# zifuwan/Sigma

Hardware: AMD Instinct MI355X
Metric: images/sec fwd+bwd sigma_small 480x640 (higher is better)
Workload: dtype f32

## Files before the change

### include/sigma_ops.h

```cpp
#ifndef SIGMA_OPS_H_
#define SIGMA_OPS_H_

#include <stdint.h>

#ifdef __cplusplus
extern "C" {
#endif

enum sigma_ops_status {
    SIGMA_OPS_OK = 0,
    SIGMA_OPS_ERR_ARG = 1,
    SIGMA_OPS_ERR_LAUNCH = 5
};

typedef struct sigma_dwconv_params {
    int32_t batch, channels, height, width;
    int32_t n_orders;
    int32_t flags;
    const float *x;
    const float *weight;
    const float *bias;
    float *out2;
    const float *g2;
    float *gpre;
// ... 79 lines not shown
    float *dbeta;
    float *workspace;
    const float *gate;
    int64_t gate_row_stride;
    float *dgate;
    int64_t dgate_row_stride;
    const float *row_scale;
    int64_t rows_per_scale;
    const float *dx_add;
} sigma_layernorm_params;

int sigma_layernorm_fwd(const sigma_layernorm_params *params, void *stream);
int sigma_layernorm_bwd(const sigma_layernorm_params *params, void *stream);
int sigma_layernorm_bwd_partial_rows(int64_t rows, int32_t channels);

typedef struct sigma_seg_accumulate_params {
    int64_t pixels;
    int32_t classes;
    int32_t first;
    const float *score;
    double *acc;
    int64_t score_plane_stride;
    int64_t acc_plane_stride;
} sigma_seg_accumulate_params;

int sigma_seg_accumulate(const sigma_seg_accumulate_params *params, void *stream);

typedef struct sigma_seg_confusion_params {
    int64_t pixels;
    int32_t classes;
// ... 19 lines not shown
```

### sigma_amd/_capi.py

```python
from __future__ import annotations

import ctypes
import os
from typing import Optional

_HERE = os.path.dirname(os.path.abspath(__file__))
LIB_PATH = os.environ.get("SIGMA_HIP_LIB") or os.path.join(_HERE, "lib", "libsigma_hip.so")

SIGMA_SCAN_ABI_VERSION = 12
SIGMA_SCAN_CHUNK = 2048
SIGMA_SCAN_CKPT_PITCH = 1280
SIGMA_SCAN_CKPT_PITCH_FINE = 640
SIGMA_SCAN_CKPT_PITCH_320 = 320
SIGMA_SCAN_CKPT_PITCH_160 = 160
SIGMA_SCAN_CKPT_PITCH_16 = 16
SIGMA_SCAN_MAX_DSTATE = 256
SIGMA_SCAN_BWD_DETERMINISTIC = 1
SIGMA_DWCONV_DETERMINISTIC = 1

DTYPE_F32, DTYPE_F16, DTYPE_BF16 = 0, 1, 2


class SigmaHipUnavailable(RuntimeError):
    pass
# ... 68 lines not shown

class LayerNormParams(ctypes.Structure):
    _fields_ = [
        ("rows", ctypes.c_int64), ("channels", ctypes.c_int32), ("eps", ctypes.c_float),
        ("x", ctypes.c_void_p), ("gamma", ctypes.c_void_p), ("beta", ctypes.c_void_p),
        ("y", ctypes.c_void_p), ("mean", ctypes.c_void_p), ("rstd", ctypes.c_void_p),
        ("dy", ctypes.c_void_p), ("dx", ctypes.c_void_p), ("dgamma", ctypes.c_void_p), ("dbeta", ctypes.c_void_p),
        ("workspace", ctypes.c_void_p),
        ("gate", ctypes.c_void_p), ("gate_row_stride", ctypes.c_int64), ("dgate", ctypes.c_void_p),
        ("dgate_row_stride", ctypes.c_int64),
        ("row_scale", ctypes.c_void_p), ("rows_per_scale", ctypes.c_int64),
        ("dx_add", ctypes.c_void_p),
    ]


class GemmParams(ctypes.Structure):
    _fields_ = [
        ("M", ctypes.c_int64), ("N", ctypes.c_int32), ("K", ctypes.c_int32),
        ("A", ctypes.c_void_p), ("Bt", ctypes.c_void_p), ("C", ctypes.c_void_p), ("bias", ctypes.c_void_p),
        ("lda", ctypes.c_int64), ("ldb", ctypes.c_int64), ("ldc", ctypes.c_int64),
        ("accumulate", ctypes.c_int32), ("batch", ctypes.c_int32),
        ("strideA", ctypes.c_int64), ("strideB", ctypes.c_int64), ("strideC", ctypes.c_int64),
        ("a_mod", ctypes.c_int32), ("pieces", ctypes.c_int32),
        ("c_mod", ctypes.c_int32), ("reserved", ctypes.c_int32),
        ("residual", ctypes.c_void_p), ("residual2", ctypes.c_void_p), ("ldr", ctypes.c_int64), ("strideR", ctypes.c_int64),
        ("Ct", ctypes.c_void_p), ("ldct", ctypes.c_int64), ("t_cols", ctypes.c_int32), ("k_slices", ctypes.c_int32),
        ("workspace", ctypes.c_void_p), ("workspace_bytes", ctypes.c_int64),
    ]


# ... 12 lines not shown
        ("score_plane_stride", ctypes.c_int64), ("acc_plane_stride", ctypes.c_int64),
    ]


class SegConfusionParams(ctypes.Structure):
    _fields_ = [
        ("pixels", ctypes.c_int64), ("classes", ctypes.c_int32), ("n_cl", ctypes.c_int32),
        ("gt_elem_size", ctypes.c_int32), ("pred_elem_size", ctypes.c_int32),
        ("acc", ctypes.c_void_p), ("acc_plane_stride", ctypes.c_int64),
        ("pred", ctypes.c_void_p), ("gt", ctypes.c_void_p), ("hist", ctypes.c_void_p), ("counts", ctypes.c_void_p),
    ]


SIGMA_CE_BLOCKS = 1024
SIGMA_SEG_LDS_HIST_BYTES = 32768

GEMM_SYMBOLS = ("sigma_gemm_nt_split3", "sigma_gemm_nn_split3", "sigma_gemm_tn_split3")
GEMM_AUX_SYMBOLS = ("sigma_gemm_selftest", "sigma_gemm_workspace_bytes", "sigma_gemm_plan")
GEMM_FORMS = {"nt": 0, "nn": 1, "tn": 2}
GEMM_EPILOGUES = ("rows", "direct", "transposed")
GEMM_RES_LOADS = ("none", "vector", "scalar")
GEMM_STORES = ("store", "accumulate", "atomic")

OPS_SYMBOLS = ("sigma_dwconv3x3_silu_fwd", "sigma_dwconv3x3_silu_bwd", "sigma_cross_merge_nhwc", "sigma_cross_split_nhwc",
               "sigma_layernorm_fwd", "sigma_layernorm_bwd", "sigma_layernorm_bwd_partial_rows", "sigma_transpose2d",
               "sigma_pair_sum_add", "sigma_upsample2x_nhwc", "sigma_plane_pool", "sigma_plane_scale",
               "sigma_plane_dot", "sigma_plane_gate_bwd", "sigma_softmax_ce_fwd", "sigma_softmax_ce_bwd", "sigma_colscale_bwd",
               "sigma_colscale_bwd_ws", "sigma_seg_accumulate", "sigma_seg_argmax_confusion")
OPS_AUX_SYMBOLS = ("sigma_dwconv3x3_silu_bwd_workspace_bytes", "sigma_colscale_bwd_workspace_bytes")

EXPORTED_SYMBOLS = (
    "sigma_selective_scan_fwd",
    "sigma_selective_scan_bwd",
    "sigma_scan_bwd_workspace_bytes",
    "sigma_scan_fwd_workspace_bytes",
    "sigma_scan_last_error",
    "sigma_scan_abi_version",
    "sigma_scan_set_option",
    "sigma_scan_get_option",
    "sigma_scan_fwd_plan",
    "sigma_scan_bwd_plan",
    "sigma_scan_selftest",
    "sigma_scan_rowlane_selftest",
)
# ... 57 lines not shown
            fn.argtypes = [ctypes.c_void_p, ctypes.c_void_p, ctypes.c_void_p, ctypes.c_void_p, ctypes.c_void_p, ctypes.c_int64,
                           ctypes.c_int32, ctypes.c_void_p]
        elif name == "sigma_colscale_bwd_ws":
            fn.argtypes = [ctypes.c_void_p, ctypes.c_void_p, ctypes.c_void_p, ctypes.c_void_p, ctypes.c_void_p, ctypes.c_int64,
                           ctypes.c_int32, ctypes.c_void_p, ctypes.c_int64, ctypes.c_void_p]
        elif name == "sigma_softmax_ce_fwd":
            fn.argtypes = [ctypes.c_void_p, ctypes.c_void_p, ctypes.c_int64, ctypes.c_int32, ctypes.c_int64, ctypes.c_void_p,
                           ctypes.c_void_p, ctypes.c_void_p]
        elif name == "sigma_softmax_ce_bwd":
            fn.argtypes = [ctypes.c_void_p, ctypes.c_void_p, ctypes.c_void_p, ctypes.c_void_p, ctypes.c_int64, ctypes.c_int32,
                           ctypes.c_int64, ctypes.c_void_p, ctypes.c_void_p]
        elif name == "sigma_seg_accumulate":
            fn.argtypes = [P(SegAccumulateParams), ctypes.c_void_p]
        elif name == "sigma_seg_argmax_confusion":
            fn.argtypes = [P(SegConfusionParams), ctypes.c_void_p]
        else:
            st = (MergeParams if "cross_" in name else LayerNormParams if "layernorm" in name else
                  TransposeParams if "transpose" in name else DwConvParams)
            fn.argtypes = [P(st), ctypes.c_void_p]
        fn.restype = ctypes.c_int
    lib.sigma_dwconv3x3_silu_bwd_workspace_bytes.argtypes = [P(DwConvParams)]
    lib.sigma_dwconv3x3_silu_bwd_workspace_bytes.restype = ctypes.c_int64
    lib.sigma_colscale_bwd_workspace_bytes.argtypes = [ctypes.c_int64, ctypes.c_int32]
    lib.sigma_colscale_bwd_workspace_bytes.restype = ctypes.c_int64
    for name in GEMM_SYMBOLS:
        fn = getattr(lib, name)
        fn.argtypes = [P(GemmParams), ctypes.c_void_p]
        fn.restype = ctypes.c_int
    lib.sigma_gemm_selftest.argtypes = [ctypes.c_void_p]
    lib.sigma_gemm_selftest.restype = ctypes.c_int
    lib.sigma_gemm_workspace_bytes.argtypes = [P(GemmParams), ctypes.c_int]
    lib.sigma_gemm_workspace_bytes.restype = ctypes.c_int64
    lib.sigma_gemm_plan.argtypes = [P(GemmParams), ctypes.c_int, P(ctypes.c_int32 * 8)]
    lib.sigma_gemm_plan.restype = ctypes.c_int
    if lib.sigma_scan_abi_version() != SIGMA_SCAN_ABI_VERSION:
        raise SigmaHipUnavailable(
            f"ABI mismatch: library {lib.sigma_scan_abi_version()} vs binding {SIGMA_SCAN_ABI_VERSION}; rebuild")
    _lib = lib
    return lib
# ... 29 lines not shown
```

### sigma_amd/build.py

```python
from __future__ import annotations

import argparse
import concurrent.futures as cf
import os
import subprocess
import sys

HERE = os.path.dirname(os.path.abspath(__file__))
CSRC = os.path.join(HERE, "csrc")
OBJ = os.path.join(HERE, "lib", "obj")
LIB = os.path.join(HERE, "lib", "libsigma_hip.so")
SOURCES = ["scan_fwd.hip", "scan_fwd4.hip", "scan_fwdr.hip", "scan_bwdr.hip", "scan_bwd.hip", "scan_bwd2.hip", "scan_bwd3.hip", "scan_bwd4.hip", "selftest.hip", "capi.hip", "dwconv.hip", "merge.hip", "layernorm.hip", "gemm_split.hip", "upsample.hip", "pointwise.hip", "segmetric.hip"]
HEADERS = ["scan_device.h", "scan_launch.h", "scan_quad.h", "scan_rowlane.h", os.path.join("..", "..", "include", "sigma_scan.h"),
           os.path.join("..", "..", "include", "sigma_ops.h"), os.path.join("..", "..", "include", "sigma_gemm.h")]
HIPCC = os.environ.get("HIPCC", "/opt/rocm/bin/hipcc")
FLAGS = [
    "--offload-arch=gfx950", "-O3", "-std=c++17", "-fPIC",
    "-munsafe-fp-atomics",
    "-ffp-contract=off",
    "-fno-slp-vectorize",
    "-Wall", "-Wno-unused-function",
]


def _newer(target: str, deps) -> bool:
    if not os.path.exists(target):
        return True
# ... 45 lines not shown
```

### sigma_amd/selective_scan_cuda_core.py

```python
from __future__ import annotations

import ctypes
from typing import List, Optional

import torch

from . import _capi

_DTYPES = {torch.float32: _capi.DTYPE_F32, torch.float16: _capi.DTYPE_F16, torch.bfloat16: _capi.DTYPE_BF16}


_launch_hook = None


def set_launch_hook(hook) -> None:
    global _launch_hook
    _launch_hook = hook


def _launch(kind, key, fn):
    return fn() if _launch_hook is None else _launch_hook(kind, key, fn)


def _check(cond: bool, msg: str) -> None:
# ... 178 lines not shown
        stream = torch.cuda.current_stream(u.device).cuda_stream
        key = (batch, dim, seqlen, dstate, sizes[4], u.element_size())
        _launch("fwd", key, lambda: _capi.check(
            lib.sigma_selective_scan_fwd(ctypes.byref(fp), ctypes.c_void_p(stream)), "selective_scan_fwd"))
    return [out, x]


def bwd(u: torch.Tensor, delta: torch.Tensor, A: torch.Tensor, B: torch.Tensor, C: torch.Tensor,
        D_: Optional[torch.Tensor], delta_bias_: Optional[torch.Tensor], dout: torch.Tensor,
        x_: Optional[torch.Tensor], delta_softplus: bool, nrows: int) -> List[Optional[torch.Tensor]]:
    return bwd_ext(u, delta, A, B, C, D_, delta_bias_, dout, x_, delta_softplus, nrows=nrows)


def bwd_ext(u, delta, A, B, C, D_, delta_bias_, dout, x_, delta_softplus, nrows: int = 1, rev_mask: int = 0,
            u_gshift: int = 0, dout_gshift: int = 0, dB_out: Optional[torch.Tensor] = None,
            dC_out: Optional[torch.Tensor] = None, ckpt_pitch: int = 0, param_swap: int = 0) -> List[Optional[torch.Tensor]]:
    lib = _capi.load()
    sizes = _check_common(u, delta, A, B, C, D_, delta_bias_, nrows, u_gshift)
    batch, dim, seqlen, dstate, n_groups = sizes
    _check(dout.dtype == u.dtype, "dout must have the dtype of u")
    _check(dout.is_cuda, "dout must be a GPU tensor")
    _check(tuple(dout.shape) == (batch, dim >> dout_gshift, seqlen), "dout must have shape (batch_size, dim, seqlen)")
    _check(dout.stride(-1) == 1 or seqlen <= 1, "dout.stride(-1) must be 1")
    if ckpt_pitch == _capi.SIGMA_SCAN_CKPT_PITCH_16 and batch > 0 and seqlen > 0 and (
            dout.data_ptr() % 16 != 0 or any(s % 4 != 0 for s in dout.stride()[:-1])):
        dout = dout.contiguous()
        if dout.data_ptr() % 16 != 0:
            dout = dout.clone()
    n_chunks = (seqlen + _capi.SIGMA_SCAN_CHUNK - 1) // _capi.SIGMA_SCAN_CHUNK
    if n_chunks > 1 or seqlen > _capi.SIGMA_SCAN_CKPT_PITCH:
        _check(x_ is not None, "x is required when seqlen > 2048")
    if x_ is not None:
        _check(x_.dtype == torch.float32 and x_.is_cuda and x_.is_contiguous(), "x must be a contiguous float32 GPU tensor")
        if x_.dim() == 3:
            pitch = _fine_pitch(x_, seqlen, dstate, ckpt_pitch)
            _check(tuple(x_.shape) == (batch, dim, _ckpt_slots(seqlen, pitch) * dstate), "fine-checkpoint x must be (batch, dim, ceil(L/pitch)*dstate)")
        else:
            _check(tuple(x_.shape) == (batch, dim, n_chunks, 2 * dstate),
                   "x must have shape (batch_size, dim, n_chunks, 2 * dstate)")
    du = torch.empty_like(delta)
    ddelta = torch.empty_like(delta)
    det = torch.are_deterministic_algorithms_enabled()
    if det and batch > 0 and seqlen > 0:
        zeros = torch.empty(dim * dstate + 2 * dim, dtype=torch.float32, device=A.device)
    else:
        zeros = torch.zeros(dim * dstate + 2 * dim, dtype=torch.float32, device=A.device)
    dA = zeros[:dim * dstate].view(dim, dstate)
    if dB_out is not None:
        _check(dB_out.dtype == torch.float32 and tuple(dB_out.shape) == tuple(B.shape) and dB_out.stride(-1) == 1 and
               dC_out is not None and dC_out.dtype == torch.float32 and tuple(dC_out.shape) == tuple(C.shape) and
               dC_out.stride(-1) == 1, "dB_out / dC_out must be fp32 views shaped like B / C")
        dB, dC = dB_out, dC_out
    elif batch > 0 and seqlen > 0:
        dB = torch.empty(B.shape, dtype=torch.float32, device=B.device)
        dC = torch.empty(C.shape, dtype=torch.float32, device=C.device)
    else:
        dB, dC = torch.zeros_like(B, dtype=torch.float32), torch.zeros_like(C, dtype=torch.float32)
    dD = zeros[dim * dstate:dim * dstate + dim] if D_ is not None else None
    ddelta_bias = zeros[dim * dstate + dim:] if delta_bias_ is not None else None
    if batch > 0 and seqlen > 0:
        bp = _capi.BwdParams()
# ... 20 lines not shown
            key = (batch, dim, seqlen, dstate, n_groups, u.element_size())
            _launch("bwd", key, lambda: _capi.check(
                lib.sigma_selective_scan_bwd(ctypes.byref(bp), ctypes.c_void_p(stream)), "selective_scan_bwd"))
            if (ckpt_pitch == _capi.SIGMA_SCAN_CKPT_PITCH_16 and lib.sigma_scan_get_option(b"rl_chain") == 2
                    and not torch.cuda.is_current_stream_capturing()):
                n = lib.sigma_scan_get_option(b"rl_chain_timeouts")
                if n != 0:
                    raise RuntimeError(
                        f"selective_scan_bwd: {n if n > 0 else 'an unknown number of'} hand-over wait(s) of the chained "
                        "row-lane walk ran out (the producer workgroup was not resident: another stream's kernel held "
                        "its slot); the gradients of this call hold NaN. Unset the 'rl_chain' option or run the scan "
                        "alone on the device")
    if dB_out is None:
        dB, dC = dB.to(B.dtype), dC.to(C.dtype)
    return [du, ddelta, dA, dB, dC, dD, ddelta_bias]
```

### sigma_amd/ss2d_fused.py

```python
from __future__ import annotations

import torch

import os as _os_early

from . import gemm as _gemm
from ._handoff import claim_xz_grad_buffer
from . import selective_scan_cuda_core as _core

_PERM = (0, 2, 1, 3)
_REV_MASK = 0b1010
_XPROJ_ALL = _os_early.environ.get("SIGMA_GEMM_XPROJ", "") == "all"
_XPROJ = 0 if _gemm.gemm_mode() == "fp32" else (2 if _XPROJ_ALL else _gemm._pieces("SIGMA_GEMM_XPROJ", "2"))


def _perm4(t: torch.Tensor) -> torch.Tensor:
    return t.unflatten(0, (2, 2)).transpose(0, 1).flatten(0, 1)
import os as _os
_CKPT_ENV = _os.environ.get("SIGMA_CKPT_PITCH", "auto")


def rowlane_possible() -> bool:
    return _CKPT_ENV in ("auto", "16")


def rowlane_pays(seqlen: int, dstate: int, rows: int, groups: int) -> bool:
    if seqlen < 600:
        return False
# ... 177 lines not shown
        if pair_sum:
            Bsz, dim, L = out.shape
            if B.shape[1] != 2:
                raise RuntimeError("pair_sum: two groups only")
            o4 = out.view(Bsz, 2, dim // 2, L)
            return o4[:, 0] + o4[:, 1]
        return out

    @staticmethod
    def backward(ctx, dout):
        u, delta, A, B, C, D, delta_bias, ck = ctx.saved_tensors
        rev_mask, sh, pair_sum = ctx.ext
        dout = dout.float()
        if dout.stride(-1) != 1:
            dout = dout.contiguous()
        du, ddelta, dA, dB, dC, dD, dbias = _core.bwd_ext(u, delta, A, B, C, D, delta_bias, dout, ck,
                                                          True, rev_mask=rev_mask, u_gshift=sh, dout_gshift=1 if pair_sum else 0,
                                                          ckpt_pitch=ctx.pitch)
        if sh:
            Bsz, dim, L = du.shape
            G = B.shape[1]
            rpg = dim // G
            du = du.view(Bsz, G >> sh, 1 << sh, rpg, L).sum(2).reshape(Bsz, dim >> sh, L)
        return du, ddelta, dA.clone(), dB, dC, dD.clone(), dbias.clone(), None, None, None


def selective_scan_ext(u, delta, A, B, C, D, delta_bias, rev_mask=0, u_gshift=0, pair_sum=False):
    return SelectiveScanExtFn.apply(u, delta, A, B, C, D, delta_bias, rev_mask, u_gshift, pair_sum)


def _merge_params(B, d, H, W):
    from . import _capi
    p = _capi.MergeParams()
    p.batch, p.channels, p.height, p.width = B, d, H, W
    return p


def cross_merge_nhwc(ys: torch.Tensor, H: int, W: int) -> torch.Tensor:
    import ctypes
# ... 93 lines not shown
        if L != H * W:
            raise RuntimeError("SS2DCoreFn: xs2 must be (B, 2, d, H*W)")
        K, c, _ = x_proj_weight.shape
        R = dt_projs_weight.shape[2]
        N = A_logs.shape[1]
        if K != 4:
            raise RuntimeError("SS2DCoreFn expects the 4-direction parameter stack")
        xs2 = xs2.float().contiguous()
        Wst, WstT, dtw, A = _derived_params(x_proj_weight, dt_projs_weight, A_logs)
        legal = bool(_XPROJ) and L % 4 == 0 and d % 4 == 0 and c % 2 == 0
        short = L <= 600 or _XPROJ_ALL
        mid = L <= 1200 or _XPROJ_ALL
        own_x = legal
        own_dt = legal and R % 4 == 0 and mid
        ctx.own = dict(xd=legal, xw=legal and mid, dd=legal and R % 4 == 0 and _XPROJ_ALL, dw=legal and R % 4 == 0 and short)
        if own_x:
            p4 = torch.empty((B, 4, c, L), device=xs2.device, dtype=torch.float32)
            _gemm.bgemm_nn(Wst, xs2.view(2 * B, d, L), p4.view(2 * B, 2 * c, L), pieces=_XPROJ)
        else:
            p4 = torch.matmul(Wst.unsqueeze(0), xs2).view(B, 4, c, L)
        if own_dt:
            delta = torch.empty((B, 4, d, L), device=xs2.device, dtype=torch.float32)
            _gemm.bgemm_nn(dtw, p4.view(4 * B, c, L)[:, :R], delta.view(4 * B, d, L), pieces=_XPROJ)
        else:
            delta = torch.matmul(dtw.unsqueeze(0), p4[:, :, :R])
        Dp = Ds.float()
        bias = dt_projs_bias.float().reshape(-1)
        Bv, Cv = p4[:, :, R:R + N], p4[:, :, R + N:]
        need_x = any(ctx.needs_input_grad)
        u2, dl2 = xs2.view(B, 2 * d, L), delta.view(B, 4 * d, L)
# ... 3 lines not shown
        ctx.pitch = pitch
        y = cross_merge_nhwc(out.view(B, 4, d, L), H, W)
        ctx.save_for_backward(xs2, p4, delta, A, Dp, bias, ck, Wst, dtw, WstT)
        ctx.dims = (B, d, H, W, c, R, N)
        return y

    @staticmethod
    def backward(ctx, dy):
        xs2, p4, delta, A, Dp, bias, ck, Wst, dtw, WstT = ctx.saved_tensors
        B, d, H, W, c, R, N = ctx.dims
        own = ctx.own
        L = H * W
        g2 = cross_split_nhwc(dy.float().contiguous())
        dp4 = torch.empty_like(p4)
        Bv, Cv = p4[:, :, R:R + N], p4[:, :, R + N:]
        du, ddelta, dA, _, _, dD, dbias = _core.bwd_ext(
            xs2.view(B, 2 * d, L), delta.view(B, 4 * d, L), A, Bv, Cv, Dp, bias, g2.view(B, 2 * d, L), ck, True,
            rev_mask=_REV_MASK, u_gshift=1, dout_gshift=1, dB_out=dp4[:, :, R:R + N], dC_out=dp4[:, :, R + N:], param_swap=1,
            ckpt_pitch=ctx.pitch)
        ddelta4 = ddelta.view(B, 4, d, L)
        wg = torch.empty(4 * d * R + 4 * c * d, device=xs2.device, dtype=torch.float32) if (own["xw"] or own["dw"]) else None
        if own["dd"]:
            _gemm.bgemm_nn(dtw.transpose(1, 2).contiguous(), ddelta.view(4 * B, d, L), dp4.view(4 * B, c, L)[:, :R], pieces=_XPROJ)
        else:
            dp4[:, :, :R] = torch.matmul(dtw.transpose(1, 2).unsqueeze(0), ddelta4)
        if own["dw"]:
            d_dtw = wg[:4 * d * R].view(4, d, R)
            _gemm.bgemm_nt_sum(ddelta.view(4 * B, d, L), p4.view(4 * B, c, L)[:, :R], d_dtw, pieces=_XPROJ, accumulate=False)
        else:
            d_dtw = torch.matmul(ddelta4, p4[:, :, :R].transpose(-1, -2)).sum(0)
        dp2 = dp4.view(B, 2, 2 * c, L)
        if own["xd"]:
            dxs2 = torch.empty((B, 2, d, L), device=xs2.device, dtype=torch.float32)
            du3 = du.view(2 * B, 2, d, L)
            _gemm.bgemm_nn(WstT, dp4.view(2 * B, 2 * c, L), dxs2.view(2 * B, d, L),
                           residual=du3[:, 0], residual2=du3[:, 1], pieces=_XPROJ)
        else:
            dxs2 = torch.matmul(WstT.unsqueeze(0), dp2)
            _pair_sum_add(du, dxs2, B * 2, d * L)
        if own["xw"]:
            dWst = wg[4 * d * R:].view(2, 2 * c, d)
            _gemm.bgemm_nt_sum(dp4.view(2 * B, 2 * c, L), xs2.view(2 * B, d, L), dWst, pieces=_XPROJ, accumulate=False)
        else:
            dWst = torch.matmul(dp2, xs2.transpose(-1, -2)).sum(0)
        d_xproj = _perm4(dWst.view(4, c, d))
        d_dtw = _perm4(d_dtw)
        dA_logs = dA * A
        dDs = dD.clone()
        dbias = dbias.clone().view(4, d)
        return dxs2, None, None, d_xproj, d_dtw, dbias, dA_logs, dDs


class _TwoOrdersFn(torch.autograd.Function):

    @staticmethod
    def forward(ctx, x):
        ctx.hw = x.shape[2:]
        return _two_orders(x.float())

    @staticmethod
    def backward(ctx, g):
        H, W = ctx.hw
        B, _, d, L = g.shape
        return g[:, 0].reshape(B, d, H, W) + g[:, 1].reshape(B, d, W, H).transpose(2, 3)

# ... 9 lines not shown
```

Measured before the change: 49.88.

## Fuse dt-projection backward GEMMs and scan parameter-grad epilogue into HIP kernels

Adds a dtproj backward kernel that computes both ddt (dtw^T·ddelta) and d_dtw (ddelta·dt^T) from a single pass over ddelta using MFMA, with a split-row reduction stage. It also adds a scan_param_grads kernel that fuses dA*A, the dD/dbias copies, the four-way permutations, and zeroing of a borrowed accumulator buffer into one launch, replacing several small torch ops and clones. The fused dtproj path is enabled only when seqlen >= 4800 by default. This adds workspace and extra code paths, and requires careful cleanup of the borrowed accumulator when an error occurs.

Result: no change. 50.21, median of 6 (+0.7%).

```diff
diff --git a/include/sigma_ops.h b/include/sigma_ops.h
--- a/include/sigma_ops.h
+++ b/include/sigma_ops.h
@@ -117,6 +117,46 @@
 int sigma_layernorm_bwd(const sigma_layernorm_params *params, void *stream);
 int sigma_layernorm_bwd_partial_rows(int64_t rows, int32_t channels);
 
+#define SIGMA_DTPROJ_LBLOCK 256
+#define SIGMA_DTPROJ_MAX_RANK 48
+#define SIGMA_DTPROJ_TARGET_WGS 1280
+typedef struct sigma_dtproj_bwd_params {
+    int32_t batch, groups, dim, seqlen;
+    int32_t rank, reserved_;
+    const float *ddelta;
+    const float *dt;
+    const float *dtw;
+    float *ddt;
+    float *d_dtw;
+    int64_t dt_batch_stride, dt_group_stride, dt_row_stride;
+    int64_t ddt_batch_stride, ddt_group_stride, ddt_row_stride;
+    void *workspace;
+    int64_t workspace_bytes;
+} sigma_dtproj_bwd_params;
+
+int sigma_dtproj_bwd(const sigma_dtproj_bwd_params *params, void *stream);
+int64_t sigma_dtproj_bwd_workspace_bytes(const sigma_dtproj_bwd_params *params);
+
+#define SIGMA_PARAM_GRADS_ZERO_ACC 1
+#define SIGMA_PARAM_GRADS_SWAP 2
+typedef struct sigma_param_grads_params {
+    int32_t dim, dstate;
+    int32_t flags;
+    int32_t n_perm;
+    float *acc_dA;
+    float *acc_dD;
+    float *acc_dbias;
+    const float *A;
+    float *dA_out;
+    float *dD_out;
+    float *dbias_out;
+    const float *perm_src[2];
+    float *perm_dst[2];
+    int64_t perm_block[2];
+} sigma_param_grads_params;
+
+int sigma_scan_param_grads(const sigma_param_grads_params *params, void *stream);
+
 typedef struct sigma_seg_accumulate_params {
     int64_t pixels;
     int32_t classes;
diff --git a/sigma_amd/_capi.py b/sigma_amd/_capi.py
--- a/sigma_amd/_capi.py
+++ b/sigma_amd/_capi.py
@@ -106,6 +106,28 @@
     ]
 
 
+class DtProjBwdParams(ctypes.Structure):
+    _fields_ = [
+        ("batch", ctypes.c_int32), ("groups", ctypes.c_int32), ("dim", ctypes.c_int32), ("seqlen", ctypes.c_int32),
+        ("rank", ctypes.c_int32), ("reserved_", ctypes.c_int32),
+        ("ddelta", ctypes.c_void_p), ("dt", ctypes.c_void_p), ("dtw", ctypes.c_void_p),
+        ("ddt", ctypes.c_void_p), ("d_dtw", ctypes.c_void_p),
+        ("dt_batch_stride", ctypes.c_int64), ("dt_group_stride", ctypes.c_int64), ("dt_row_stride", ctypes.c_int64),
+        ("ddt_batch_stride", ctypes.c_int64), ("ddt_group_stride", ctypes.c_int64), ("ddt_row_stride", ctypes.c_int64),
+        ("workspace", ctypes.c_void_p), ("workspace_bytes", ctypes.c_int64),
+    ]
+
+
+class ParamGradsParams(ctypes.Structure):
+    _fields_ = [
+        ("dim", ctypes.c_int32), ("dstate", ctypes.c_int32), ("flags", ctypes.c_int32), ("n_perm", ctypes.c_int32),
+        ("acc_dA", ctypes.c_void_p), ("acc_dD", ctypes.c_void_p), ("acc_dbias", ctypes.c_void_p),
+        ("A", ctypes.c_void_p),
+        ("dA_out", ctypes.c_void_p), ("dD_out", ctypes.c_void_p), ("dbias_out", ctypes.c_void_p),
+        ("perm_src", ctypes.c_void_p * 2), ("perm_dst", ctypes.c_void_p * 2), ("perm_block", ctypes.c_int64 * 2),
+    ]
+
+
 class GemmParams(ctypes.Structure):
     _fields_ = [
         ("M", ctypes.c_int64), ("N", ctypes.c_int32), ("K", ctypes.c_int32),
@@ -148,6 +170,10 @@
 
 SIGMA_CE_BLOCKS = 1024
 SIGMA_SEG_LDS_HIST_BYTES = 32768
+SIGMA_DTPROJ_LBLOCK = 256
+SIGMA_DTPROJ_MAX_RANK = 48
+SIGMA_DTPROJ_TARGET_WGS = 1280
+SIGMA_PARAM_GRADS_ZERO_ACC, SIGMA_PARAM_GRADS_SWAP = 1, 2
 
 GEMM_SYMBOLS = ("sigma_gemm_nt_split3", "sigma_gemm_nn_split3", "sigma_gemm_tn_split3")
 GEMM_AUX_SYMBOLS = ("sigma_gemm_selftest", "sigma_gemm_workspace_bytes", "sigma_gemm_plan")
@@ -160,8 +186,10 @@
                "sigma_layernorm_fwd", "sigma_layernorm_bwd", "sigma_layernorm_bwd_partial_rows", "sigma_transpose2d",
                "sigma_pair_sum_add", "sigma_upsample2x_nhwc", "sigma_plane_pool", "sigma_plane_scale",
                "sigma_plane_dot", "sigma_plane_gate_bwd", "sigma_softmax_ce_fwd", "sigma_softmax_ce_bwd", "sigma_colscale_bwd",
-               "sigma_colscale_bwd_ws", "sigma_seg_accumulate", "sigma_seg_argmax_confusion")
-OPS_AUX_SYMBOLS = ("sigma_dwconv3x3_silu_bwd_workspace_bytes", "sigma_colscale_bwd_workspace_bytes")
+               "sigma_colscale_bwd_ws", "sigma_seg_accumulate", "sigma_seg_argmax_confusion", "sigma_dtproj_bwd",
+               "sigma_scan_param_grads")
+OPS_AUX_SYMBOLS = ("sigma_dwconv3x3_silu_bwd_workspace_bytes", "sigma_colscale_bwd_workspace_bytes",
+                   "sigma_dtproj_bwd_workspace_bytes")
 
 EXPORTED_SYMBOLS = (
     "sigma_selective_scan_fwd",
@@ -249,6 +277,10 @@
             fn.argtypes = [P(SegAccumulateParams), ctypes.c_void_p]
         elif name == "sigma_seg_argmax_confusion":
             fn.argtypes = [P(SegConfusionParams), ctypes.c_void_p]
+        elif name == "sigma_dtproj_bwd":
+            fn.argtypes = [P(DtProjBwdParams), ctypes.c_void_p]
+        elif name == "sigma_scan_param_grads":
+            fn.argtypes = [P(ParamGradsParams), ctypes.c_void_p]
         else:
             st = (MergeParams if "cross_" in name else LayerNormParams if "layernorm" in name else
                   TransposeParams if "transpose" in name else DwConvParams)
@@ -258,6 +290,8 @@
     lib.sigma_dwconv3x3_silu_bwd_workspace_bytes.restype = ctypes.c_int64
     lib.sigma_colscale_bwd_workspace_bytes.argtypes = [ctypes.c_int64, ctypes.c_int32]
     lib.sigma_colscale_bwd_workspace_bytes.restype = ctypes.c_int64
+    lib.sigma_dtproj_bwd_workspace_bytes.argtypes = [P(DtProjBwdParams)]
+    lib.sigma_dtproj_bwd_workspace_bytes.restype = ctypes.c_int64
     for name in GEMM_SYMBOLS:
         fn = getattr(lib, name)
         fn.argtypes = [P(GemmParams), ctypes.c_void_p]
diff --git a/sigma_amd/build.py b/sigma_amd/build.py
--- a/sigma_amd/build.py
+++ b/sigma_amd/build.py
@@ -10,7 +10,7 @@
 CSRC = os.path.join(HERE, "csrc")
 OBJ = os.path.join(HERE, "lib", "obj")
 LIB = os.path.join(HERE, "lib", "libsigma_hip.so")
-SOURCES = ["scan_fwd.hip", "scan_fwd4.hip", "scan_fwdr.hip", "scan_bwdr.hip", "scan_bwd.hip", "scan_bwd2.hip", "scan_bwd3.hip", "scan_bwd4.hip", "selftest.hip", "capi.hip", "dwconv.hip", "merge.hip", "layernorm.hip", "gemm_split.hip", "upsample.hip", "pointwise.hip", "segmetric.hip"]
+SOURCES = ["scan_fwd.hip", "scan_fwd4.hip", "scan_fwdr.hip", "scan_bwdr.hip", "scan_bwd.hip", "scan_bwd2.hip", "scan_bwd3.hip", "scan_bwd4.hip", "selftest.hip", "capi.hip", "dwconv.hip", "merge.hip", "layernorm.hip", "gemm_split.hip", "upsample.hip", "pointwise.hip", "segmetric.hip", "dtproj.hip"]
 HEADERS = ["scan_device.h", "scan_launch.h", "scan_quad.h", "scan_rowlane.h", os.path.join("..", "..", "include", "sigma_scan.h"),
            os.path.join("..", "..", "include", "sigma_ops.h"), os.path.join("..", "..", "include", "sigma_gemm.h")]
 HIPCC = os.environ.get("HIPCC", "/opt/rocm/bin/hipcc")
diff --git a/sigma_amd/csrc/dtproj.hip b/sigma_amd/csrc/dtproj.hip
--- /dev/null
+++ b/sigma_amd/csrc/dtproj.hip
@@ -0,0 +1,339 @@
+#include <hip/hip_runtime.h>
+#include <stdint.h>
+
+#include "../../include/sigma_ops.h"
+
+namespace sigma {
+namespace {
+
+typedef float f32x4 __attribute__((ext_vector_type(4)));
+
+constexpr int LB = SIGMA_DTPROJ_LBLOCK;
+constexpr int WL = LB / 4;
+constexpr int DT = 32;
+constexpr int PITCH = LB + 4;
+
+struct DtArgs {
+    const float* ddelta;
+    const float* dt;
+    const float* dtw;
+    float* ddt;
+    float* ws;
+    float* part;
+    long dt_bs, dt_gs, dt_rs, ddt_bs, ddt_gs, ddt_rs;
+    int B, G, d, L, R, nlb, nseg, seg_rows;
+};
+
+__device__ __forceinline__ float4 ldg4(const float* p) { return *reinterpret_cast<const float4*>(p); }
+
+template <int RT>
+__global__ void __launch_bounds__(256) dtproj_bwd_kernel(const DtArgs a) {
+    __shared__ __attribute__((aligned(16))) float xs[DT * PITCH];
+    __shared__ __attribute__((aligned(16))) float red[4 * DT * RT * 16];
+    constexpr int RP = RT * 16;
+    const int tid = threadIdx.x, wave = tid >> 6, lane = tid & 63, i = lane & 15, q = lane >> 4;
+    const int lb = blockIdx.x, g = blockIdx.y / a.nseg, seg = blockIdx.y - g * a.nseg, b = blockIdx.z;
+    const int L = a.L, R = a.R;
+    const int dbeg = seg * a.seg_rows;
+    const int d = dbeg + a.seg_rows < a.d ? dbeg + a.seg_rows : a.d;
+    const int l0 = lb * LB, lw = wave * WL;
+    const float* X = a.ddelta + ((long)b * a.G + g) * (long)a.d * L;
+    const float* W = a.dtw + (long)g * a.d * R;
+
+    float4 dtr[RT][4];
+    {
+        const float* dtp = a.dt + b * a.dt_bs + g * a.dt_gs;
+#pragma unroll
+        for (int rt = 0; rt < RT; ++rt)
+#pragma unroll
+            for (int m = 0; m < 4; ++m) {
+                const int r = 16 * rt + i, l = l0 + lw + 16 * m + 4 * q;
+                dtr[rt][m] = (r < R && l < L) ? ldg4(dtp + r * a.dt_rs + l) : make_float4(0.f, 0.f, 0.f, 0.f);
+            }
+    }
+    f32x4 acc1[RT][4];
+#pragma unroll
+    for (int rt = 0; rt < RT; ++rt)
+#pragma unroll
+        for (int e = 0; e < 4; ++e) acc1[rt][e] = f32x4{0.f, 0.f, 0.f, 0.f};
+
+    const int srow = tid >> 6, scol = 4 * (tid & 63);
+    const bool col_ok = l0 + scol < L;
+    float4 pf[8];
+    auto fetch = [&](int d0) {
+#pragma unroll
+        for (int p = 0; p < 8; ++p) {
+            const int row = d0 + 4 * p + srow;
+            pf[p] = (col_ok && row < d) ? ldg4(X + (long)row * L + l0 + scol) : make_float4(0.f, 0.f, 0.f, 0.f);
+        }
+    };
+    float wn[8][RT];
+    auto fetch_w = [&](int d0) {
+#pragma unroll
+        for (int s = 0; s < 8; ++s)
+#pragma unroll
+            for (int rt = 0; rt < RT; ++rt) {
+                const int dd = d0 + 4 * s + q, r = 16 * rt + i;
+                wn[s][rt] = (dd < d && r < R) ? W[(long)dd * R + r] : 0.f;
+            }
+    };
+    fetch(dbeg);
+    fetch_w(dbeg);
+    float* slot = a.ws + (((long)b * a.nlb + lb) * a.G + g) * (long)a.d * R;
+    const bool wave_on = l0 + lw < L;
+
+    for (int d0 = dbeg; d0 < d; d0 += DT) {
+#pragma unroll
+        for (int p = 0; p < 8; ++p) *reinterpret_cast<float4*>(xs + (4 * p + srow) * PITCH + scol) = pf[p];
+        float wr[8][RT];
+#pragma unroll
+        for (int s = 0; s < 8; ++s)
+#pragma unroll
+            for (int rt = 0; rt < RT; ++rt) wr[s][rt] = wn[s][rt];
+        __syncthreads();
+        if (d0 + DT < d) {
+            fetch(d0 + DT);
+            fetch_w(d0 + DT);
+        }
+
+        if (wave_on)
+#pragma unroll
+        for (int s = 0; s < 8; ++s) {
+            const float4 x = *reinterpret_cast<const float4*>(xs + (4 * s + q) * PITCH + lw + 4 * i);
+            const float xe[4] = {x.x, x.y, x.z, x.w};
+#pragma unroll
+            for (int rt = 0; rt < RT; ++rt)
+#pragma unroll
+                for (int e = 0; e < 4; ++e) acc1[rt][e] = __builtin_amdgcn_mfma_f32_16x16x4f32(wr[s][rt], xe[e], acc1[rt][e], 0, 0, 0);
+        }
+        f32x4 acc2[2][RT];
+#pragma unroll
+        for (int u = 0; u < 2; ++u)
+#pragma unroll
+            for (int rt = 0; rt < RT; ++rt) acc2[u][rt] = f32x4{0.f, 0.f, 0.f, 0.f};
+        if (wave_on)
+#pragma unroll
+        for (int m = 0; m < 4; ++m) {
+            const float4 x0 = *reinterpret_cast<const float4*>(xs + i * PITCH + lw + 16 * m + 4 * q);
+            const float4 x1 = *reinterpret_cast<const float4*>(xs + (16 + i) * PITCH + lw + 16 * m + 4 * q);
+            const float xe[2][4] = {{x0.x, x0.y, x0.z, x0.w}, {x1.x, x1.y, x1.z, x1.w}};
+#pragma unroll
+            for (int e = 0; e < 4; ++e)
+#pragma unroll
+                for (int u = 0; u < 2; ++u)
+#pragma unroll
+                    for (int rt = 0; rt < RT; ++rt) {
+                        const float4 t = dtr[rt][m];
+                        const float te = e == 0 ? t.x : e == 1 ? t.y : e == 2 ? t.z : t.w;
+                        acc2[u][rt] = __builtin_amdgcn_mfma_f32_16x16x4f32(xe[u][e], te, acc2[u][rt], 0, 0, 0);
+                    }
+        }
+#pragma unroll
+        for (int u = 0; u < 2; ++u)
+#pragma unroll
+            for (int rt = 0; rt < RT; ++rt)
+#pragma unroll
+                for (int k = 0; k < 4; ++k) red[(wave * DT + 16 * u + 4 * q + k) * RP + 16 * rt + i] = acc2[u][rt][k];
+        __syncthreads();
+        const int rows = d - d0 < DT ? d - d0 : DT;
+        for (int idx = tid; idx < rows * R; idx += 256) {
+            const int dl = idx / R, r = idx - dl * R;
+            const int o = dl * RP + r;
+            slot[(long)d0 * R + idx] = ((red[o] + red[DT * RP + o]) + red[2 * DT * RP + o]) + red[3 * DT * RP + o];
+        }
+    }
+
+    const int l = l0 + lw + 4 * i;
+    if (l < L) {
+        float* out = a.ddt + b * a.ddt_bs + g * a.ddt_gs + l;
+        long rs = a.ddt_rs;
+        if (a.nseg > 1) {
+            out = a.part + (((long)seg * a.B + b) * a.G + g) * (long)R * L + l;
+            rs = L;
+        }
+#pragma unroll
+        for (int rt = 0; rt < RT; ++rt)
+#pragma unroll
+            for (int k = 0; k < 4; ++k) {
+                const int r = 16 * rt + 4 * q + k;
+                if (r < R)
+                    *reinterpret_cast<float4*>(out + r * rs) = make_float4(acc1[rt][0][k], acc1[rt][1][k], acc1[rt][2][k], acc1[rt][3][k]);
+            }
+    }
+}
+
+__global__ void __launch_bounds__(256) dtproj_reduce_kernel(const float* __restrict__ ws, float* __restrict__ out, int slots, long n4,
+                                                            int dw_blocks, const DtArgs a) {
+    if ((int)blockIdx.x >= dw_blocks) {
+        const long L4 = a.L >> 2, per = (long)a.B * a.G * a.R * L4;
+        const long t = (long)(blockIdx.x - dw_blocks) * 256 + threadIdx.x;
+        if (t >= per) return;
+        float4 acc = ldg4(a.part + t * 4);
+        for (int s = 1; s < a.nseg; ++s) {
+            const float4 v = ldg4(a.part + ((long)s * per + t) * 4);
+            acc.x += v.x; acc.y += v.y; acc.z += v.z; acc.w += v.w;
+        }
+        const long row = t / L4, l4 = t - row * L4;
+        const long bg = row / a.R, r = row - bg * a.R, b = bg / a.G, g = bg - b * a.G;
+        *reinterpret_cast<float4*>(a.ddt + b * a.ddt_bs + g * a.ddt_gs + r * a.ddt_rs + 4 * l4) = acc;
+        return;
+    }
+    __shared__ float4 part[4][64];
+    const int x = threadIdx.x & 63, y = threadIdx.x >> 6;
+    const long c = (long)blockIdx.x * 64 + x;
+    float4 acc = make_float4(0.f, 0.f, 0.f, 0.f);
+    if (c < n4)
+        for (int s = y; s < slots; s += 4) {
+            const float4 v = ldg4(ws + ((long)s * n4 + c) * 4);
+            acc.x += v.x; acc.y += v.y; acc.z += v.z; acc.w += v.w;
+        }
+    part[y][x] = acc;
+    __syncthreads();
+    if (y == 0 && c < n4) {
+        float4 t = part[0][x];
+        for (int k = 1; k < 4; ++k) { t.x += part[k][x].x; t.y += part[k][x].y; t.z += part[k][x].z; t.w += part[k][x].w; }
+        *reinterpret_cast<float4*>(out + c * 4) = t;
+    }
+}
+
+struct PgArgs {
+    float* acc_dA; float* acc_dD; float* acc_dbias;
+    const float* A;
+    float* dA_out; float* dD_out; float* dbias_out;
+    const float* perm_src[2];
+    float* perm_dst[2];
+    long perm_block[2];
+    long nA, dim;
+    int zero, swap;
+};
+
+__global__ void __launch_bounds__(256) scan_param_grads_kernel(const PgArgs a) {
+    const long n1 = a.nA, n2 = n1 + (a.acc_dD ? a.dim : 0), n3 = n2 + (a.acc_dbias ? a.dim : 0);
+    const long n4 = n3 + 4 * a.perm_block[0], n5 = n4 + 4 * a.perm_block[1];
+    for (long t = (long)blockIdx.x * 256 + threadIdx.x; t < n5; t += (long)gridDim.x * 256) {
+        if (t < n1) {
+            const float v = a.acc_dA[t];
+            a.dA_out[t] = a.A ? v * a.A[t] : v;
+            if (a.zero) a.acc_dA[t] = 0.f;
+        } else if (t < n2) {
+            a.dD_out[t - n1] = a.acc_dD[t - n1];
+            if (a.zero) a.acc_dD[t - n1] = 0.f;
+        } else if (t < n3) {
+            a.dbias_out[t - n2] = a.acc_dbias[t - n2];
+            if (a.zero) a.acc_dbias[t - n2] = 0.f;
+        } else {
+            const int p = t < n4 ? 0 : 1;
+            const long o = t - (p ? n4 : n3), pb = a.perm_block[p];
+            const long k = o / pb, r = o - k * pb;
+            const long ks = (a.swap && (k == 1 || k == 2)) ? 3 - k : k;
+            a.perm_dst[p][o] = a.perm_src[p][ks * pb + r];
+        }
+    }
+}
+
+bool al16(const void* p) { return (reinterpret_cast<uintptr_t>(p) & 15u) == 0; }
+
+constexpr int64_t LIM = (int64_t)1 << 31;
+
+int64_t extent(const sigma_dtproj_bwd_params* p, int64_t bs, int64_t gs, int64_t rs) {
+    return (p->batch - 1) * bs + (p->groups - 1) * gs + (p->rank - 1) * rs + p->seqlen;
+}
+
+int64_t dt_slots(const sigma_dtproj_bwd_params* p) { return (int64_t)p->batch * ((p->seqlen + LB - 1) / LB); }
+
+bool dt_sizes_ok(const sigma_dtproj_bwd_params* p) {
+    if (!p || p->batch < 1 || p->groups < 1 || p->dim < 1 || p->seqlen < 4 || p->rank < 4) return false;
+    if (p->rank % 4 != 0 || p->rank > SIGMA_DTPROJ_MAX_RANK || p->seqlen % 4 != 0) return false;
+    if (p->batch > 65535 || p->groups > 1024) return false;
+    if ((int64_t)p->batch * p->groups * p->dim * p->seqlen >= LIM) return false;
+    if ((int64_t)p->groups * p->dim * p->rank >= LIM) return false;
+    if (dt_slots(p) * p->groups * p->dim * p->rank >= LIM) return false;
+    return true;
+}
+
+void dt_segments(const sigma_dtproj_bwd_params* p, int* nseg, int* seg_rows) {
+    const int tiles = (p->dim + DT - 1) / DT;
+    const int64_t wgs = dt_slots(p) * p->groups;
+    int64_t want = (SIGMA_DTPROJ_TARGET_WGS + wgs - 1) / wgs;
+    if (want > tiles / 4) want = tiles / 4;
+    if (want < 1) want = 1;
+    const int seg_tiles = (int)((tiles + want - 1) / want);
+    *nseg = (tiles + seg_tiles - 1) / seg_tiles;
+    *seg_rows = seg_tiles * DT;
+}
+
+}
+}
+
+extern "C" {
+
+int64_t sigma_dtproj_bwd_workspace_bytes(const sigma_dtproj_bwd_params* p) {
+    if (!sigma::dt_sizes_ok(p)) return -1;
+    int nseg, seg_rows;
+    sigma::dt_segments(p, &nseg, &seg_rows);
+    const int64_t parts = nseg > 1 ? (int64_t)nseg * p->batch * p->groups * p->rank * p->seqlen : 0;
+    return (sigma::dt_slots(p) * p->groups * p->dim * p->rank + parts) * (int64_t)sizeof(float);
+}
+
+int sigma_dtproj_bwd(const sigma_dtproj_bwd_params* p, void* stream) {
+    using namespace sigma;
+    if (!dt_sizes_ok(p)) return SIGMA_OPS_ERR_ARG;
+    if (!p->ddelta || !p->dt || !p->dtw || !p->ddt || !p->d_dtw || !p->workspace) return SIGMA_OPS_ERR_ARG;
+    if (!al16(p->ddelta) || !al16(p->dt) || !al16(p->dtw) || !al16(p->ddt) || !al16(p->d_dtw) || !al16(p->workspace)) return SIGMA_OPS_ERR_ARG;
+    const int64_t strides[6] = {p->dt_batch_stride, p->dt_group_stride, p->dt_row_stride,
+                                p->ddt_batch_stride, p->ddt_group_stride, p->ddt_row_stride};
+    for (int64_t s : strides)
+        if (s < 0 || s % 4 != 0 || s >= LIM) return SIGMA_OPS_ERR_ARG;
+    if (p->dt_row_stride < p->seqlen || p->ddt_row_stride < p->seqlen) return SIGMA_OPS_ERR_ARG;
+    if (extent(p, p->dt_batch_stride, p->dt_group_stride, p->dt_row_stride) >= LIM ||
+        extent(p, p->ddt_batch_stride, p->ddt_group_stride, p->ddt_row_stride) >= LIM) return SIGMA_OPS_ERR_ARG;
+    const int64_t need = sigma_dtproj_bwd_workspace_bytes(p);
+    if (p->workspace_bytes < need) return SIGMA_OPS_ERR_ARG;
+    const int nlb = (p->seqlen + LB - 1) / LB;
+    int nseg, seg_rows;
+    dt_segments(p, &nseg, &seg_rows);
+    float* ws = static_cast<float*>(p->workspace);
+    DtArgs a{p->ddelta, p->dt, p->dtw, p->ddt, ws, ws + dt_slots(p) * p->groups * p->dim * p->rank,
+             (long)p->dt_batch_stride, (long)p->dt_group_stride, (long)p->dt_row_stride,
+             (long)p->ddt_batch_stride, (long)p->ddt_group_stride, (long)p->ddt_row_stride,
+             p->batch, p->groups, p->dim, p->seqlen, p->rank, nlb, nseg, seg_rows};
+    hipStream_t st = static_cast<hipStream_t>(stream);
+    const dim3 grid((unsigned)nlb, (unsigned)(p->groups * nseg), (unsigned)p->batch);
+    const int rt = (p->rank + 15) / 16;
+    if (rt == 1) hipLaunchKernelGGL(dtproj_bwd_kernel<1>, grid, dim3(256), 0, st, a);
+    else if (rt == 2) hipLaunchKernelGGL(dtproj_bwd_kernel<2>, grid, dim3(256), 0, st, a);
+    else hipLaunchKernelGGL(dtproj_bwd_kernel<3>, grid, dim3(256), 0, st, a);
+    if (hipGetLastError() != hipSuccess) return SIGMA_OPS_ERR_LAUNCH;
+    const long n4 = (long)p->groups * p->dim * p->rank / 4;
+    const long dw_blocks = (n4 + 63) / 64;
+    const long ddt_blocks = nseg > 1 ? ((long)p->batch * p->groups * p->rank * (p->seqlen / 4) + 255) / 256 : 0;
+    hipLaunchKernelGGL(dtproj_reduce_kernel, dim3((unsigned)(dw_blocks + ddt_blocks)), dim3(256), 0, st, static_cast<const float*>(p->workspace),
+                       p->d_dtw, (int)dt_slots(p), n4, (int)dw_blocks, a);
+    return hipGetLastError() == hipSuccess ? SIGMA_OPS_OK : SIGMA_OPS_ERR_LAUNCH;
+}
+
+int sigma_scan_param_grads(const sigma_param_grads_params* p, void* stream) {
+    using namespace sigma;
+    if (!p || p->dim < 1 || p->dstate < 1 || p->n_perm < 0 || p->n_perm > 2) return SIGMA_OPS_ERR_ARG;
+    if (p->flags & ~(SIGMA_PARAM_GRADS_ZERO_ACC | SIGMA_PARAM_GRADS_SWAP)) return SIGMA_OPS_ERR_ARG;
+    if (!p->acc_dA || !p->dA_out) return SIGMA_OPS_ERR_ARG;
+    if ((p->acc_dD == nullptr) != (p->dD_out == nullptr) || (p->acc_dbias == nullptr) != (p->dbias_out == nullptr)) return SIGMA_OPS_ERR_ARG;
+    PgArgs a{};
+    a.acc_dA = p->acc_dA; a.acc_dD = p->acc_dD; a.acc_dbias = p->acc_dbias; a.A = p->A;
+    a.dA_out = p->dA_out; a.dD_out = p->dD_out; a.dbias_out = p->dbias_out;
+    a.nA = (long)p->dim * p->dstate; a.dim = p->dim;
+    a.zero = (p->flags & SIGMA_PARAM_GRADS_ZERO_ACC) ? 1 : 0;
+    a.swap = (p->flags & SIGMA_PARAM_GRADS_SWAP) ? 1 : 0;
+    long total = a.nA + (a.acc_dD ? a.dim : 0) + (a.acc_dbias ? a.dim : 0);
+    for (int k = 0; k < p->n_perm; ++k) {
+        if (!p->perm_src[k] || !p->perm_dst[k] || p->perm_block[k] < 1 || p->perm_block[k] >= LIM / 4) return SIGMA_OPS_ERR_ARG;
+        a.perm_src[k] = p->perm_src[k]; a.perm_dst[k] = p->perm_dst[k]; a.perm_block[k] = (long)p->perm_block[k];
+        total += 4 * a.perm_block[k];
+    }
+    long blocks = (total + 255) / 256;
+    if (blocks > 1024) blocks = 1024;
+    hipLaunchKernelGGL(scan_param_grads_kernel, dim3((unsigned)blocks), dim3(256), 0, static_cast<hipStream_t>(stream), a);
+    return hipGetLastError() == hipSuccess ? SIGMA_OPS_OK : SIGMA_OPS_ERR_LAUNCH;
+}
+
+}
diff --git a/sigma_amd/selective_scan_cuda_core.py b/sigma_amd/selective_scan_cuda_core.py
--- a/sigma_amd/selective_scan_cuda_core.py
+++ b/sigma_amd/selective_scan_cuda_core.py
@@ -216,7 +216,8 @@
 
 def bwd_ext(u, delta, A, B, C, D_, delta_bias_, dout, x_, delta_softplus, nrows: int = 1, rev_mask: int = 0,
             u_gshift: int = 0, dout_gshift: int = 0, dB_out: Optional[torch.Tensor] = None,
-            dC_out: Optional[torch.Tensor] = None, ckpt_pitch: int = 0, param_swap: int = 0) -> List[Optional[torch.Tensor]]:
+            dC_out: Optional[torch.Tensor] = None, ckpt_pitch: int = 0, param_swap: int = 0,
+            borrow_acc: bool = False) -> List[Optional[torch.Tensor]]:
     lib = _capi.load()
     sizes = _check_common(u, delta, A, B, C, D_, delta_bias_, nrows, u_gshift)
     batch, dim, seqlen, dstate, n_groups = sizes
@@ -246,7 +247,9 @@
     if det and batch > 0 and seqlen > 0:
         zeros = torch.empty(dim * dstate + 2 * dim, dtype=torch.float32, device=A.device)
     else:
-        zeros = torch.zeros(dim * dstate + 2 * dim, dtype=torch.float32, device=A.device)
+        zeros = _acc_buffer(dim * dstate + 2 * dim, A.device) if borrow_acc else None
+        if zeros is None:
+            zeros = torch.zeros(dim * dstate + 2 * dim, dtype=torch.float32, device=A.device)
     dA = zeros[:dim * dstate].view(dim, dstate)
     if dB_out is not None:
         _check(dB_out.dtype == torch.float32 and tuple(dB_out.shape) == tuple(B.shape) and dB_out.stride(-1) == 1 and
@@ -297,3 +300,108 @@
     if dB_out is None:
         dB, dC = dB.to(B.dtype), dC.to(C.dtype)
     return [du, ddelta, dA, dB, dC, dD, ddelta_bias]
+
+
+_ACC = {}
+_ACC_RETIRED = []
+_ACC_MIN_FLOATS = 1 << 18
+
+
+def _acc_key(device):
+    dev = torch.device(device)
+    idx = dev.index if dev.index is not None else torch.cuda.current_device()
+    return idx, torch.cuda.current_stream(dev).cuda_stream
+
+
+def _acc_buffer(n: int, device) -> Optional[torch.Tensor]:
+    key = _acc_key(device)
+    buf = _ACC.get(key)
+    if buf is None or buf.numel() < n:
+        if torch.cuda.is_current_stream_capturing():
+            return None
+        if buf is not None:
+            _ACC_RETIRED.append(buf)
+        buf = torch.zeros(max(n, _ACC_MIN_FLOATS), dtype=torch.float32, device=device)
+        _ACC[key] = buf
+    return buf[:n]
+
+
+def drop_acc_buffer(device=None) -> None:
+    keys = list(_ACC) if device is None else [_acc_key(device)]
+    for key in keys:
+        buf = _ACC.pop(key, None)
+        if buf is not None:
+            _ACC_RETIRED.append(buf)
+
+
+def is_acc_view(t: torch.Tensor) -> bool:
+    buf = _ACC.get(_acc_key(t.device)) if t.is_cuda else None
+    return buf is not None and t.untyped_storage().data_ptr() == buf.untyped_storage().data_ptr()
+
+
+def scan_param_grads(dA, dD, dbias, A=None, perm=(), swap: bool = False):
+    lib = _capi.load()
+    _check(dA.is_cuda and dA.dtype == torch.float32 and dA.dim() == 2 and dA.is_contiguous(), "scan_param_grads: dA must be a contiguous fp32 (dim, dstate) GPU tensor")
+    dim, dstate = dA.shape
+    p = _capi.ParamGradsParams()
+    p.dim, p.dstate, p.n_perm = dim, dstate, len(perm)
+    _check(len(perm) <= 2, "scan_param_grads: at most two permuted copies")
+    p.flags = (_capi.SIGMA_PARAM_GRADS_ZERO_ACC if is_acc_view(dA) else 0) | (_capi.SIGMA_PARAM_GRADS_SWAP if swap else 0)
+    outs = [torch.empty_like(dA)]
+    p.acc_dA, p.dA_out = dA.data_ptr(), outs[0].data_ptr()
+    if A is not None:
+        _check(A.dtype == torch.float32 and tuple(A.shape) == (dim, dstate) and A.is_contiguous() and A.device == dA.device,
+               "scan_param_grads: A must be fp32, contiguous, shaped like dA")
+        p.A = A.data_ptr()
+    for name, t in (("dD", dD), ("dbias", dbias)):
+        if t is None:
+            outs.append(None)
+            continue
+        _check(t.dtype == torch.float32 and tuple(t.shape) == (dim,) and t.is_contiguous() and t.device == dA.device,
+               f"scan_param_grads: {name} must be fp32 (dim)")
+        outs.append(torch.empty_like(t))
+        setattr(p, "acc_" + name, t.data_ptr())
+        setattr(p, name + "_out", outs[-1].data_ptr())
+    keep = []
+    for k, t in enumerate(perm):
+        _check(t.dtype == torch.float32 and t.dim() >= 1 and t.shape[0] == 4 and t.device == dA.device and t.numel() > 0,
+               "scan_param_grads: permuted tensors must be fp32 (4, ...)")
+        t = t.contiguous()
+        keep.append(t)
+        outs.append(torch.empty_like(t))
+        p.perm_src[k], p.perm_dst[k], p.perm_block[k] = t.data_ptr(), outs[-1].data_ptr(), t.numel() // 4
+    with torch.cuda.device(dA.device):
+        _capi.check(lib.sigma_scan_param_grads(ctypes.byref(p), ctypes.c_void_p(torch.cuda.current_stream(dA.device).cuda_stream)),
+                    "scan_param_grads")
+    return outs
+
+
+def dtproj_bwd_ok(rank: int, seqlen: int) -> bool:
+    return rank % 4 == 0 and 4 <= rank <= _capi.SIGMA_DTPROJ_MAX_RANK and seqlen % 4 == 0 and seqlen >= 4
+
+
+def dtproj_bwd(ddelta, dt, dtw, ddt, d_dtw=None):
+    lib = _capi.load()
+    B, G, d, L = ddelta.shape
+    R = dtw.shape[2]
+    for name, t in (("ddelta", ddelta), ("dt", dt), ("dtw", dtw), ("ddt", ddt)):
+        _check(t.is_cuda and t.dtype == torch.float32, f"dtproj_bwd: {name} must be an fp32 GPU tensor")
+    _check(ddelta.is_contiguous() and dtw.is_contiguous() and tuple(dtw.shape) == (G, d, R), "dtproj_bwd: ddelta (B, G, d, L) and dtw (G, d, R) must be contiguous")
+    _check(tuple(dt.shape) == (B, G, R, L) and tuple(ddt.shape) == (B, G, R, L) and dt.stride(-1) == 1 and ddt.stride(-1) == 1,
+           "dtproj_bwd: dt / ddt must be (B, G, R, L) with unit inner stride")
+    if d_dtw is None:
+        d_dtw = torch.empty((G, d, R), dtype=torch.float32, device=ddelta.device)
+    _check(tuple(d_dtw.shape) == (G, d, R) and d_dtw.is_contiguous() and d_dtw.dtype == torch.float32, "dtproj_bwd: d_dtw must be fp32 (G, d, R) contiguous")
+    p = _capi.DtProjBwdParams()
+    p.batch, p.groups, p.dim, p.seqlen, p.rank = B, G, d, L, R
+    p.ddelta, p.dt, p.dtw, p.ddt, p.d_dtw = ddelta.data_ptr(), dt.data_ptr(), dtw.data_ptr(), ddt.data_ptr(), d_dtw.data_ptr()
+    p.dt_batch_stride, p.dt_group_stride, p.dt_row_stride = dt.stride(0), dt.stride(1), dt.stride(2)
+    p.ddt_batch_stride, p.ddt_group_stride, p.ddt_row_stride = ddt.stride(0), ddt.stride(1), ddt.stride(2)
+    ws_bytes = int(lib.sigma_dtproj_bwd_workspace_bytes(ctypes.byref(p)))
+    _check(ws_bytes >= 0, "dtproj_bwd: sizes the kernel cannot take (rank % 4, rank <= 48, seqlen % 4, 31-bit offsets)")
+    workspace = torch.empty(max(ws_bytes, 16), dtype=torch.uint8, device=ddelta.device)
+    p.workspace, p.workspace_bytes = workspace.data_ptr(), ws_bytes
+    with torch.cuda.device(ddelta.device):
+        rc = lib.sigma_dtproj_bwd(ctypes.byref(p), ctypes.c_void_p(torch.cuda.current_stream(ddelta.device).cuda_stream))
+    _check(rc == 0, f"dtproj_bwd: refused (sigma_ops_status {rc}): alignment, strides or sizes")
+    return d_dtw
diff --git a/sigma_amd/ss2d_fused.py b/sigma_amd/ss2d_fused.py
--- a/sigma_amd/ss2d_fused.py
+++ b/sigma_amd/ss2d_fused.py
@@ -12,6 +12,11 @@
 _REV_MASK = 0b1010
 _XPROJ_ALL = _os_early.environ.get("SIGMA_GEMM_XPROJ", "") == "all"
 _XPROJ = 0 if _gemm.gemm_mode() == "fp32" else (2 if _XPROJ_ALL else _gemm._pieces("SIGMA_GEMM_XPROJ", "2"))
+_DTPROJ_FUSED = _os_early.environ.get("SIGMA_DTPROJ_BWD", "table")
+
+
+def dtproj_fused_pays(seqlen: int) -> bool:
+    return seqlen >= 4800
 
 
 def _perm4(t: torch.Tensor) -> torch.Tensor:
@@ -219,15 +224,20 @@
         dout = dout.float()
         if dout.stride(-1) != 1:
             dout = dout.contiguous()
-        du, ddelta, dA, dB, dC, dD, dbias = _core.bwd_ext(u, delta, A, B, C, D, delta_bias, dout, ck,
-                                                          True, rev_mask=rev_mask, u_gshift=sh, dout_gshift=1 if pair_sum else 0,
-                                                          ckpt_pitch=ctx.pitch)
+        try:
+            du, ddelta, dA, dB, dC, dD, dbias = _core.bwd_ext(u, delta, A, B, C, D, delta_bias, dout, ck,
+                                                              True, rev_mask=rev_mask, u_gshift=sh, dout_gshift=1 if pair_sum else 0,
+                                                              ckpt_pitch=ctx.pitch, borrow_acc=True)
+            dA, dD, dbias = _core.scan_param_grads(dA, dD, dbias)
+        except BaseException:
+            _core.drop_acc_buffer(u.device)
+            raise
         if sh:
             Bsz, dim, L = du.shape
             G = B.shape[1]
             rpg = dim // G
             du = du.view(Bsz, G >> sh, 1 << sh, rpg, L).sum(2).reshape(Bsz, dim >> sh, L)
-        return du, ddelta, dA.clone(), dB, dC, dD.clone(), dbias.clone(), None, None, None
+        return du, ddelta, dA, dB, dC, dD, dbias, None, None, None
 
 
 def selective_scan_ext(u, delta, A, B, C, D, delta_bias, rev_mask=0, u_gshift=0, pair_sum=False):
@@ -351,6 +361,8 @@
         own_x = legal
         own_dt = legal and R % 4 == 0 and mid
         ctx.own = dict(xd=legal, xw=legal and mid, dd=legal and R % 4 == 0 and _XPROJ_ALL, dw=legal and R % 4 == 0 and short)
+        ctx.own["dt_fused"] = (legal and not _XPROJ_ALL and _core.dtproj_bwd_ok(R, L) and
+                               (_DTPROJ_FUSED == "all" or (_DTPROJ_FUSED == "table" and dtproj_fused_pays(L))))
         if own_x:
             p4 = torch.empty((B, 4, c, L), device=xs2.device, dtype=torch.float32)
             _gemm.bgemm_nn(Wst, xs2.view(2 * B, d, L), p4.view(2 * B, 2 * c, L), pieces=_XPROJ)
@@ -384,21 +396,39 @@
         g2 = cross_split_nhwc(dy.float().contiguous())
         dp4 = torch.empty_like(p4)
         Bv, Cv = p4[:, :, R:R + N], p4[:, :, R + N:]
-        du, ddelta, dA, _, _, dD, dbias = _core.bwd_ext(
-            xs2.view(B, 2 * d, L), delta.view(B, 4 * d, L), A, Bv, Cv, Dp, bias, g2.view(B, 2 * d, L), ck, True,
-            rev_mask=_REV_MASK, u_gshift=1, dout_gshift=1, dB_out=dp4[:, :, R:R + N], dC_out=dp4[:, :, R + N:], param_swap=1,
-            ckpt_pitch=ctx.pitch)
+        try:
+            du, ddelta, dA, _, _, dD, dbias = _core.bwd_ext(
+                xs2.view(B, 2 * d, L), delta.view(B, 4 * d, L), A, Bv, Cv, Dp, bias, g2.view(B, 2 * d, L), ck, True,
+                rev_mask=_REV_MASK, u_gshift=1, dout_gshift=1, dB_out=dp4[:, :, R:R + N], dC_out=dp4[:, :, R + N:], param_swap=1,
+                ckpt_pitch=ctx.pitch, borrow_acc=True)
+            dxs2, dWst, d_dtw = SS2DCoreFn._projection_grads(ctx, xs2, p4, dp4, du, ddelta, Wst, dtw, WstT)
+            dA_logs, dDs, dbias, d_xproj, d_dtw = _core.scan_param_grads(dA, dD, dbias, A=A, perm=(dWst.view(4, c, d), d_dtw),
+                                                                         swap=True)
+        except BaseException:
+            _core.drop_acc_buffer(xs2.device)
+            raise
+        return dxs2, None, None, d_xproj, d_dtw, dbias.view(4, d), dA_logs, dDs
+
+    @staticmethod
+    def _projection_grads(ctx, xs2, p4, dp4, du, ddelta, Wst, dtw, WstT):
+        B, d, H, W, c, R, N = ctx.dims
+        own = ctx.own
+        L = H * W
         ddelta4 = ddelta.view(B, 4, d, L)
-        wg = torch.empty(4 * d * R + 4 * c * d, device=xs2.device, dtype=torch.float32) if (own["xw"] or own["dw"]) else None
-        if own["dd"]:
-            _gemm.bgemm_nn(dtw.transpose(1, 2).contiguous(), ddelta.view(4 * B, d, L), dp4.view(4 * B, c, L)[:, :R], pieces=_XPROJ)
+        wg = (torch.empty(4 * d * R + 4 * c * d, device=xs2.device, dtype=torch.float32)
+              if (own["xw"] or own["dw"] or own["dt_fused"]) else None)
+        if own["dt_fused"]:
+            d_dtw = _core.dtproj_bwd(ddelta4, p4[:, :, :R], dtw, dp4[:, :, :R], wg[:4 * d * R].view(4, d, R))
         else:
-            dp4[:, :, :R] = torch.matmul(dtw.transpose(1, 2).unsqueeze(0), ddelta4)
-        if own["dw"]:
-            d_dtw = wg[:4 * d * R].view(4, d, R)
-            _gemm.bgemm_nt_sum(ddelta.view(4 * B, d, L), p4.view(4 * B, c, L)[:, :R], d_dtw, pieces=_XPROJ, accumulate=False)
-        else:
-            d_dtw = torch.matmul(ddelta4, p4[:, :, :R].transpose(-1, -2)).sum(0)
+            if own["dd"]:
+                _gemm.bgemm_nn(dtw.transpose(1, 2).contiguous(), ddelta.view(4 * B, d, L), dp4.view(4 * B, c, L)[:, :R], pieces=_XPROJ)
+            else:
+                dp4[:, :, :R] = torch.matmul(dtw.transpose(1, 2).unsqueeze(0), ddelta4)
+            if own["dw"]:
+                d_dtw = wg[:4 * d * R].view(4, d, R)
+                _gemm.bgemm_nt_sum(ddelta.view(4 * B, d, L), p4.view(4 * B, c, L)[:, :R], d_dtw, pieces=_XPROJ, accumulate=False)
+            else:
+                d_dtw = torch.matmul(ddelta4, p4[:, :, :R].transpose(-1, -2)).sum(0)
         dp2 = dp4.view(B, 2, 2 * c, L)
         if own["xd"]:
             dxs2 = torch.empty((B, 2, d, L), device=xs2.device, dtype=torch.float32)
@@ -413,12 +443,7 @@
             _gemm.bgemm_nt_sum(dp4.view(2 * B, 2 * c, L), xs2.view(2 * B, d, L), dWst, pieces=_XPROJ, accumulate=False)
         else:
             dWst = torch.matmul(dp2, xs2.transpose(-1, -2)).sum(0)
-        d_xproj = _perm4(dWst.view(4, c, d))
-        d_dtw = _perm4(d_dtw)
-        dA_logs = dA * A
-        dDs = dD.clone()
-        dbias = dbias.clone().view(4, d)
-        return dxs2, None, None, d_xproj, d_dtw, dbias, dA_logs, dDs
+        return dxs2, dWst, d_dtw
 
 
 class _TwoOrdersFn(torch.autograd.Function):
```
